# lisanhu/LongReadMapper

Measured on AMD Instinct MI355X. Metric: aligned Gbp/sec, higher is better.
Workload: dtype u8/u64 integer; 1 GPU; E. coli K-12 sized synthetic reference (4641652 bp, 5% planted repeats), 100000 x 10000 bp ont-profile reads per GPU; seed_len=20, thres=300, gact_T=320, gact_O=120, gact_W=128, reads_per_gpu=100000, read_len=10000, streams=3, sa_sampled=1, parallelism=reads sharded, index replicated (1 RCCL bcast)

## Files before the change

longreadmapper_amd/csrc/index_image.hip:

```cpp
#include <hip/hip_runtime.h>
#include <cstdio>
#include <cstdlib>
#include <cstring>
#include <new>
#include <vector>
#include <algorithm>
#include <omp.h>
#include "lrm_hip_util.h"
#include "extend_stage.h"

static inline uint64_t align256(uint64_t x) { return (x + 255ull) & ~255ull; }
#define LRM_LCX_MAX 4096

enum { S_OCC, S_LC, S_LCX, S_SA, S_CONTENT, S_MTA, N_SECTIONS };
struct Section { uint64_t LrmBlobHeader::*off; uint64_t elem; uint64_t (*count)(const LrmBlobHeader &); };
static const Section k_sections[N_SECTIONS] = {
    {&LrmBlobHeader::off_occ, sizeof(LrmOccBlock), [](const LrmBlobHeader &h) { return h.n_blocks; }},
    {&LrmBlobHeader::off_lc, 8, [](const LrmBlobHeader &h) { return h.lc_entries; }},
    {&LrmBlobHeader::off_lcx, 24, [](const LrmBlobHeader &) { return (uint64_t) LRM_LCX_MAX; }},
    {&LrmBlobHeader::off_sa, 8, [](const LrmBlobHeader &h) { return h.sa_len; }},
    {&LrmBlobHeader::off_content, 1, [](const LrmBlobHeader &h) { return h.con_len + 1; }},
    {&LrmBlobHeader::off_mta, sizeof(LrmMtaDev), [](const LrmBlobHeader &h) { return (uint64_t) (h.mta_len > 0 ? h.mta_len : 1); }},
};
static inline uint64_t section_bytes(const LrmBlobHeader &h, int s) { return k_sections[s].elem * k_sections[s].count(h); }
// ... 357 lines not shown
                                const char *content, uint64_t con_len, const lrm_mta_entry *mta, int mta_len, int device) {
    return lrm_index_upload_one(out, fmi, lch, sa, content, con_len, mta, mta_len, device, nullptr);
}

extern "C" int lrm_index_pack_device(const lrm_dna_fmi *fmi, const lrm_lc_hash *lch, const lrm_sa_mem *sa,
                                     const char *content, uint64_t con_len, const lrm_mta_entry *mta, int mta_len,
                                     void *d_blob, uint64_t blob_bytes, int device) {
    return lrm_index_pack_device_opt(fmi, lch, sa, content, con_len, mta, mta_len, d_blob, blob_bytes, device, nullptr);
}
extern "C" int lrm_index_pack_device_opt(const lrm_dna_fmi *fmi, const lrm_lc_hash *lch, const lrm_sa_mem *sa,
                                         const char *content, uint64_t con_len, const lrm_mta_entry *mta, int mta_len,
                                         void *d_blob, uint64_t blob_bytes, int device, const lrm_index_options *opt) {
    if (!fmi || !lch || !d_blob) { lrm_set_error("null argument"); return -1; }
    if (lrm_require_device(device)) return -1;
    BlobPacker pk;
    if (pk.init(fmi, lch, sa, content, con_len, mta, mta_len, opt)) return -1;
    if (blob_bytes < pk.h.total_bytes) { lrm_set_error("device buffer too small for the image"); return -1; }
    return stream_image(pk, d_blob);
}

extern "C" int lrm_index_get_tables(const lrm_index *idx, lrm_index_tables *out) {
    if (!idx || !out) { lrm_set_error("lrm_index_get_tables: null argument"); return -1; }
    memset(out, 0, sizeof(*out));
    const LrmIndexView &v = idx->view;
    uint64_t bytes = 0;
    if (v.lcl) {
        out->lc_long = v.hl; out->lc_pair = v.lcl_pair; out->lc_entry_bytes = v.lcl_kbits ? 5 : 8;
        bytes += ((v.lcl_pair ? 2ull : 1ull) << (2 * v.hl)) * (uint64_t) out->lc_entry_bytes;
        if (v.lclx) bytes += (v.lclx_mask + 1) * 16;
    }
    if (v.core) { out->lc_core = 1; bytes += 64ull << 26; }
    if (v.sd) {
        out->seed_table_len = v.sd_len; out->seed_table_share = v.sd_f; out->seed_table_bits = v.sd_bits;
        out->seed_table_slot_bytes = v.sd_slot; out->seed_table_count_bits = v.sd_cbits;
        out->seed_table_side_entries = idx->sd_side_entries;
        bytes += (64ull << v.sd_bits) + (v.sdx_mask + 1) * 16;
    }
    out->derived_bytes = bytes;
    return 0;
}

extern "C" void lrm_index_free(lrm_index *idx) {
    if (!idx) return;
    for (int r = 1; r < idx->n_peers && idx->peers; ++r) lrm_index_free(idx->peers[r]);
    delete[] idx->peers;
    (void) hipSetDevice(idx->device);
    lrm_host_ctx_free(idx);
    lrm_bs_free_index(idx);
    if (idx->d_lcl) (void) hipFree(idx->d_lcl);
    if (idx->d_lclx) (void) hipFree(idx->d_lclx);
    if (idx->d_core) (void) hipFree(idx->d_core);
    if (idx->d_sd) (void) hipFree(idx->d_sd);
    if (idx->d_sdx) (void) hipFree(idx->d_sdx);
    if (idx->owns_blob && idx->d_blob) (void) hipFree(idx->d_blob);
    delete idx;
}
```

longreadmapper_amd/csrc/index_tables.hip:

```cpp
#include <hip/hip_runtime.h>
#include <cstdio>
#include "seed_index_dev.h"

__device__ __forceinline__ uint64_t lcl_entry(const LrmIndexView &ix, int hl, uint64_t code) {
    const int ext = hl - ix.hlen;
    uint64_t k, l;
    lc_lookup(ix, code >> (2 * ext), k, l);
    if (k == 0 && l == 0) return 0;
    for (int i = ext - 1; i >= 0 && k <= l; --i) {
        const uint32_t c = (uint32_t) (code >> (2 * i)) & 3u;
        uint64_t ra, rb;
        occ_lf2(ix, c, k - 1, l, ra, rb);
        k = ra + 1;
        l = rb;
    }
    if (k > l) return 0;
    const uint64_t cnt = l - k + 1;
    return cnt >= 0xFFFFFFull ? (0xFFFFFFull << 40) : (k | (cnt << 40));
}

__global__ __launch_bounds__(256) void lcl_build_kernel(LrmIndexView ix, int hl, int pair, int kbits, uint64_t *__restrict__ out,
                                                        uint64_t slot0, uint64_t *__restrict__ ovf, uint64_t ovf_cap,
                                                        unsigned long long *__restrict__ n_ovf) {
    const uint64_t slot = slot0 + (uint64_t) blockIdx.x * 256 + threadIdx.x;
// ... 105 lines not shown
            const uint32_t at = atomicAdd(reinterpret_cast<uint32_t *>(line) + 15, 1u) & 0xFFu;
            if (at >= 250u) atomicAdd(n_ovf, 1ull << 40);
            if (at >= 10u) atomicOr(reinterpret_cast<uint32_t *>(line) + 15, 1u << (8u + sd_filter_bit((uint32_t) key.tag)));
            if (at < 10u) {
                uint16_t *h = reinterpret_cast<uint16_t *>(line) + 3 * at;
                h[0] = (uint16_t) v; h[1] = (uint16_t) (v >> 16); h[2] = (uint16_t) (v >> 32);
                placed = true;
            }
        }
        if (!placed) to_side = true;
    }
    if (to_side) {
        const unsigned long long at = atomicAdd(n_ovf, 1ull);
        if (at < ovf_cap) { ovf[2 * at] = code; ovf[2 * at + 1] = side; }
    }
}

__global__ __launch_bounds__(256) void sd_clear_kernel(ulonglong2 *__restrict__ p, uint64_t n16) {
    for (uint64_t i = (uint64_t) blockIdx.x * 256 + threadIdx.x; i < n16; i += (uint64_t) gridDim.x * 256) p[i] = make_ulonglong2(0, 0);
}

struct SdPlan { int f, bits, slot, kbits, cbits; uint64_t bytes; };
static bool sd_plan(const lrm_index *idx, uint64_t free_b, SdPlan *pl) {
    const LrmIndexTune &tu = idx->itune;
    const uint64_t L = idx->view.length;
    const int S = tu.sd_len;
    if (tu.sd == 0 || !idx->cpl_ok || L < 64 || idx->view.con_len != L) return false;
    int kbits = 1;
    while ((1ull << kbits) < L) ++kbits;
    for (int f = 4; f >= 2; f -= 2) {
        if (tu.sd_f && tu.sd_f != f) continue;
        const int slot = f == 4 ? 8 : 6, lf = f == 4 ? 2 : 1;
        const double target = f == 4 ? 2.2 : 6.0;
        int bits = 10;
        while ((double) f * (double) L / (double) (1ull << bits) > target && bits < 34) ++bits;
        if (tu.sd_bits) bits = tu.sd_bits;
        const int CL2 = 2 * (S - f + 1);
        if (bits > CL2) bits = CL2;
        if (bits < 11) bits = 11;
        if (bits < CL2 - 31) bits = CL2 - 31;
        const int tb = lf + 2 * (f - 1) + (CL2 - bits);
        int cbits = (slot == 8 ? 63 : 48) - tb - kbits;
        if (cbits < (tu.sd_bits ? 2 : 4) || tb > 40) continue;
        if (cbits > 24) cbits = 24;
        if (tu.sd_cbits && tu.sd_cbits < cbits) cbits = tu.sd_cbits;
        const uint64_t bytes = 64ull << bits;
        const uint64_t spare = bytes >= (32ull << 30) ? (40ull << 30) : (8ull << 30);
        if (tu.sd < 0 && ((uint64_t) free_b < bytes + bytes / 8 + spare || (tu.lc_long_max >= 13 && bytes > (16ull << 30)))) continue;
        pl->f = f; pl->bits = bits; pl->slot = slot; pl->kbits = kbits; pl->cbits = cbits; pl->bytes = bytes;
        return true;
    }
    return false;
}
static int sd_build(lrm_index *idx, const SdPlan &pl) {
    uint64_t *d = nullptr, *ovf = nullptr, *tab = nullptr;
    uint32_t *claimed = nullptr;
    unsigned long long *n_ovf = nullptr;
    const char *why = "";
    unsigned long long n = 0;
    auto give_up = [&]() {
        if (idx->mtune.verbose) fprintf(stderr, "[lrm] seed table (share %d, 2^%d lines, %d-byte slots) not built: %s (side entries %llu)\n", pl.f, pl.bits, pl.slot, why, n);
        if (d) (void) hipFree(d); if (ovf) (void) hipFree(ovf); if (tab) (void) hipFree(tab); if (n_ovf) (void) hipFree(n_ovf);
        if (claimed) (void) hipFree(claimed);
        (void) hipGetLastError(); return 0; };
    const uint64_t L = idx->view.length, lines = 1ull << pl.bits;
    uint64_t ovf_cap = lines / 4 + 4096;
    if (ovf_cap > (1ull << 30)) ovf_cap = 1ull << 30;
    if (idx->itune.sd_bits) ovf_cap = (uint64_t) pl.f * L + 4096;
    why = "no room for the table";
    if (hipMalloc(&d, pl.bytes) != hipSuccess) { d = nullptr; return give_up(); }
    why = "no room for the overflow list";
    if (hipMalloc(&ovf, ovf_cap * 16) != hipSuccess) { ovf = nullptr; return give_up(); }
    if (hipMalloc(&n_ovf, 8) != hipSuccess) { n_ovf = nullptr; return give_up(); }
    const uint64_t cl_bytes = ((L + 31) / 32 + 1) * 4;
    if (hipMalloc(&claimed, cl_bytes) != hipSuccess) { claimed = nullptr; return give_up(); }
    why = "memset failed";
    if (hipMemset(claimed, 0, cl_bytes) != hipSuccess) return give_up();
    hipLaunchKernelGGL(sd_clear_kernel, dim3(256 * 64), dim3(256), 0, 0, reinterpret_cast<ulonglong2 *>(d), pl.bytes / 16);
    if (hipGetLastError() != hipSuccess || hipMemset(n_ovf, 0, 8) != hipSuccess) return give_up();
    LrmIndexView sdv = idx->view;
    sdv.sd_len = idx->itune.sd_len; sdv.sd_f = pl.f; sdv.sd_bits = pl.bits; sdv.sd_kbits = pl.kbits; sdv.sd_slot = pl.slot; sdv.sd_cbits = pl.cbits;
    const uint64_t chunk = 1ull << 22;
    for (uint64_t b0 = 0, blocks = (L + 255) / 256; b0 < blocks; b0 += chunk) {
        const uint64_t nb = blocks - b0 < chunk ? blocks - b0 : chunk;
        hipLaunchKernelGGL(sd_build_kernel, dim3((uint32_t) nb), dim3(256), 0, 0, idx->view, sdv, d, b0 * 256, claimed, ovf, ovf_cap, n_ovf);
    }
    why = "build kernel failed";
    if (hipDeviceSynchronize() != hipSuccess) { give_up(); lrm_set_error("seed table build failed"); return -1; }
    why = "too many entries beside their lines";
    if (hipMemcpy(&n, n_ovf, 8, hipMemcpyDeviceToHost) != hipSuccess || n > ovf_cap) return give_up();
    uint64_t tslots = 1024;
    while (tslots < 2 * n) tslots <<= 1;
    why = "no room for the side table";
    if (hipMalloc(&tab, tslots * 16) != hipSuccess) { tab = nullptr; return give_up(); }
    if (hipMemset(tab, 0, tslots * 16) != hipSuccess) return give_up();
    if (n) hipLaunchKernelGGL(lclx_build_kernel, dim3((uint32_t) ((n + 255) / 256)), dim3(256), 0, 0, ovf, (uint64_t) n, tab, tslots - 1);
    if (hipDeviceSynchronize() != hipSuccess) { give_up(); lrm_set_error("seed table side build failed"); return -1; }
    (void) hipFree(ovf); (void) hipFree(n_ovf); (void) hipFree(claimed);
    idx->d_sd = d; idx->d_sdx = tab;
    idx->view.sd = d; idx->view.sdx = tab; idx->view.sdx_mask = tslots - 1;
    idx->view.sd_len = sdv.sd_len; idx->view.sd_f = pl.f; idx->view.sd_bits = pl.bits; idx->view.sd_kbits = pl.kbits; idx->view.sd_slot = pl.slot;
    idx->view.sd_cbits = pl.cbits;
    idx->sd_side_entries = n;
    if (idx->mtune.verbose) fprintf(stderr, "[lrm] seed table: %d positions per line, 2^%d lines, %d-byte slots, %d count bits, %llu side entries\n", pl.f, pl.bits, pl.slot, pl.cbits, n);
    return 0;
}

static int lcl_prepare_tables(lrm_index *idx, size_t free_b, bool have_sd);
int lrm_lcl_prepare_index(lrm_index *idx) {
    size_t free_b = 0, total_b = 0;
    if (hipMemGetInfo(&free_b, &total_b) != hipSuccess) { (void) hipGetLastError(); free_b = 0; }
    SdPlan sdp;
    const bool want_sd = sd_plan(idx, free_b, &sdp);
    if (want_sd) { const uint64_t need = sdp.bytes + sdp.bytes / 8; free_b = free_b > need ? free_b - need : 0; }
    const int rc_lcl = lcl_prepare_tables(idx, free_b, want_sd);
    if (rc_lcl) return rc_lcl;
    return want_sd ? sd_build(idx, sdp) : 0;
}

static int lcl_prepare_tables(lrm_index *idx, size_t free_b, bool have_sd) {
    const uint64_t L = idx->view.length;
    int hl = 13, pair = 1, ebytes = 8;
    int kbits = 1;
    while ((1ull << kbits) < L) ++kbits;
    static const struct { int hl, ebytes; uint64_t spare, min_rows; } ladder[] = {
        {17, 5, 40ull << 30, 1ull << 32}, {16, 8, 64ull << 30, 0}, {15, 8, 32ull << 30, 0}, {14, 8, 8ull << 30, 0}};
    for (const auto &c : ladder)
        if (L >= c.min_rows && kbits <= 36 && !(have_sd && c.hl > 16) && (uint64_t) free_b >= (2ull * c.ebytes << (2 * c.hl)) + c.spare) { hl = c.hl; ebytes = c.ebytes; break; }
    const LrmIndexTune &tu = idx->itune;
    if (tu.lc_long_max >= 13 && hl > tu.lc_long_max) { hl = tu.lc_long_max; ebytes = 8; }
    if (tu.lc_long >= 0) { if (tu.lc_long != hl) ebytes = 8; hl = tu.lc_long; }
    if (tu.lc_pair >= 0) pair = tu.lc_pair != 0;
    if (tu.lc_entry_bytes) ebytes = tu.lc_entry_bytes;
    if (!pair || kbits > 36) ebytes = 8;
    if (tu.lc_count_bits && 40 - tu.lc_count_bits >= kbits) kbits = 40 - tu.lc_count_bits;
    if (hl <= idx->view.hlen || hl > 17 || L < 2) return 0;
    uint64_t *d = nullptr, *ovf = nullptr, *tab = nullptr;
    unsigned long long *n_ovf = nullptr;
    const uint64_t slots = (pair ? 2ull : 1ull) << (2 * hl);
    const uint64_t ovf_cap = ebytes == 5 ? (slots / 64 < (64ull << 20) ? slots / 64 + 1024 : (64ull << 20)) : 0;
    auto give_up = [&]() { if (d) (void) hipFree(d); if (ovf) (void) hipFree(ovf); if (tab) (void) hipFree(tab); if (n_ovf) (void) hipFree(n_ovf); (void) hipGetLastError(); };
    if (hipMalloc(&d, slots * (uint64_t) ebytes + 16) != hipSuccess) { d = nullptr; give_up(); return 0; }
    if (ebytes == 5 && (hipMalloc(&ovf, ovf_cap * 16) != hipSuccess || hipMalloc(&n_ovf, 8) != hipSuccess || hipMemset(n_ovf, 0, 8) != hipSuccess)) { give_up(); return 0; }
    const uint64_t chunk = 1ull << 22;
    for (uint64_t b0 = 0, blocks = slots / 256; b0 < blocks; b0 += chunk) {
        const uint64_t nb = blocks - b0 < chunk ? blocks - b0 : chunk;
        hipLaunchKernelGGL(lcl_build_kernel, dim3((uint32_t) nb), dim3(256), 0, 0, idx->view, hl, pair, ebytes == 5 ? kbits : 0, d, b0 * 256,
                           ovf, ovf_cap, n_ovf);
    }
    if (hipDeviceSynchronize() != hipSuccess) { give_up(); lrm_set_error("long lc table build failed"); return -1; }
    uint64_t mask = 0;
    if (ebytes == 5) {
        unsigned long long n = 0;
        if (hipMemcpy(&n, n_ovf, 8, hipMemcpyDeviceToHost) != hipSuccess || n > ovf_cap) { give_up(); return 0; }
        uint64_t tslots = 1024;
        while (tslots < 2 * n) tslots <<= 1;
        mask = tslots - 1;
        if (hipMalloc(&tab, tslots * 16) != hipSuccess || hipMemset(tab, 0, tslots * 16) != hipSuccess) { give_up(); return 0; }
// ... 39 lines not shown
```

longreadmapper_amd/csrc/lrm_api.hip:

```cpp
#include <hip/hip_runtime.h>
#include <cstdarg>
#include <cstdio>
#include <cstdlib>
#include <cstring>
#include <algorithm>
#include <vector>
#include <sched.h>
#include <omp.h>
#include "lrm_hip_util.h"
#include "extend_stage.h"
#include "aln_diff_step.h"
#include "rival_rule.h"

static thread_local char g_err[512] = "";

void lrm_set_error(const char *fmt, ...) {
    va_list ap;
    va_start(ap, fmt);
    vsnprintf(g_err, sizeof(g_err), fmt, ap);
    va_end(ap);
}

extern "C" const char *lrm_last_error(void) { return g_err; }
int lrm_host_threads(void) {
    static const int cap = []() {
        int m = 1 << 20;
        cpu_set_t set;
        if (sched_getaffinity(0, sizeof(set), &set) == 0) { const int c = CPU_COUNT(&set); if (c >= 1 && c < m) m = c; }
        long long quota = -1, period = 0;
        if (FILE *f = fopen("/sys/fs/cgroup/cpu.max", "r")) {
            char q[64];
            if (fscanf(f, "%63s %lld", q, &period) == 2 && strcmp(q, "max") != 0) quota = atoll(q);
            fclose(f);
        } else {
            FILE *fq = fopen("/sys/fs/cgroup/cpu/cpu.cfs_quota_us", "r"), *fp = fopen("/sys/fs/cgroup/cpu/cpu.cfs_period_us", "r");
            if (fq && fp && fscanf(fq, "%lld", &quota) == 1 && fscanf(fp, "%lld", &period) == 1) {} else quota = -1;
            if (fq) fclose(fq);
            if (fp) fclose(fp);
        }
        if (quota > 0 && period > 0) { const int c = (int) (quota / period); if (c >= 1 && c < m) m = c; }
        return m < 1 ? 1 : m;
    }();
    const int m = omp_get_max_threads();
    const int n = m < cap ? m : cap;
    return n < 1 ? 1 : n;
}

extern "C" int lrm_abi_version(void) { return LRM_ABI_VERSION; }

extern "C" int lrm_device_count(void) {
    int n = 0;
    if (hipGetDeviceCount(&n) != hipSuccess) return 0;
    return n;
}

static const char *const k_env_names[] = {
    "LRM_SA_SAMPLED", "LRM_LC_LONG", "LRM_LC_PAIR", "LRM_LC_BYTES", "LRM_LC_CORE", "LRM_LCX_THRESHOLD", "LRM_SD", "LRM_SD_SHARE", "LRM_SD_BITS",
    "LRM_GACT_IMPL", "LRM_SEED_ROUNDS", "LRM_HOST_DENSE", "LRM_HOST_SLICE", "LRM_HOST_SUBS",
    "LRM_HOST_GROUP", "LRM_BS_WAVES", "LRM_SS_ITEMS", "LRM_VOTE_VG", "LRM_VOTE_T1", "LRM_VOTE_U", "LRM_VOTE_LOAD",
    "LRM_HOST_EXT_STREAMS", "LRM_HOST_SEED_STREAMS", "LRM_HOST_VERBOSE", "LRM_VOTE_FAST", "LRM_HOST_SLOTS", "LRM_SS_PAD"};
static_assert(sizeof(k_env_names) / sizeof(k_env_names[0]) <= LrmEnv::MAXV, "LrmEnv too small");

void lrm_env_snapshot(LrmEnv *e) {
    e->n = 0;
    for (const char *name : k_env_names)
        if (const char *v = getenv(name)) {
            e->name[e->n] = name;
            e->val[e->n] = *v ? strtoll(v, nullptr, 0) : 1;
            e->n++;
        }
}
bool LrmEnv::get(const char *key, long long *out) const {
    for (int i = 0; i < n; ++i) if (strcmp(name[i], key) == 0) { *out = val[i]; return true; }
    return false;
}

extern "C" void lrm_index_options_init(lrm_index_options *o) {
    if (!o) return;
    memset(o, 0, sizeof(*o));
    o->struct_size = (uint32_t) sizeof(*o);
    o->lc_long = -1;
    o->lc_pair = -1;
    o->lc_core = -1;
    o->seed_table = -1;
}
extern "C" void lrm_map_options_init(lrm_map_options *o) {
    if (!o) return;
    memset(o, 0, sizeof(*o));
    o->struct_size = (uint32_t) sizeof(*o);
}

static inline bool valid_sa_ratio(long long r) { return r >= 2 && r <= 64 && (r & (r - 1)) == 0; }

void lrm_resolve_index_tune(const lrm_index_options *opt, const LrmEnv &env, LrmIndexTune *t) {
    lrm_index_options o;
    lrm_index_options_init(&o);
    lrm_options_over_defaults(&o, opt);
    t->sa_ratio = valid_sa_ratio(o.sa_sampled) ? o.sa_sampled : 1;
    t->lc_long = o.lc_long; t->lc_long_max = o.lc_long_max; t->lc_pair = o.lc_pair;
    t->lc_entry_bytes = o.lc_entry_bytes == 5 || o.lc_entry_bytes == 8 ? (int) o.lc_entry_bytes : 0;
    t->lc_count_bits = o.lc_count_bits >= 2 && o.lc_count_bits <= 24 ? (int) o.lc_count_bits : 0;
    t->lc_core = o.lc_core;
    t->sd = o.seed_table;
    t->sd_len = o.seed_table_len >= 16 && o.seed_table_len <= 24 ? (int) o.seed_table_len : 20;
    t->sd_f = o.seed_table_share == 2 || o.seed_table_share == 4 ? (int) o.seed_table_share : 0;
    t->sd_bits = o.seed_table_bits >= 4 && o.seed_table_bits <= 32 ? (int) o.seed_table_bits : 0;
    t->sd_cbits = o.seed_table_count_bits >= 2 && o.seed_table_count_bits <= 24 ? (int) o.seed_table_count_bits : 0;
    t->lcx_threshold = o.lcx_threshold >= 1 && o.lcx_threshold <= 0xFFFFFFu ? o.lcx_threshold : 0xFFFFFFull;
    long long v;
    if (env.get("LRM_SA_SAMPLED", &v)) t->sa_ratio = valid_sa_ratio(v) ? (int) v : 1;
    if (env.get("LRM_LC_LONG", &v)) t->lc_long = (int) v;
    if (env.get("LRM_LC_PAIR", &v)) t->lc_pair = v != 0;
    if (env.get("LRM_LC_BYTES", &v) && (v == 5 || v == 8)) t->lc_entry_bytes = (int) v;
    if (env.get("LRM_LC_CORE", &v)) t->lc_core = v != 0;
    if (env.get("LRM_SD", &v)) t->sd = v != 0;
    if (env.get("LRM_SD_SHARE", &v) && (v == 2 || v == 4)) t->sd_f = (int) v;
    if (env.get("LRM_SD_BITS", &v) && v >= 4 && v <= 32) t->sd_bits = (int) v;
    if (env.get("LRM_LCX_THRESHOLD", &v) && v >= 1 && v <= 0xFFFFFFll) t->lcx_threshold = (uint64_t) v;
}

void lrm_resolve_map_tune(const lrm_map_options *opt, const LrmEnv &env, LrmMapTune *t) {
    lrm_map_options o;
    lrm_map_options_init(&o);
    lrm_options_over_defaults(&o, opt);
    memset(t, 0, sizeof(*t));
    t->cigar_text = o.cigar_text != 0;
    t->dense = o.dense_results != 0 || t->cigar_text;
    t->gact_impl = o.gact_impl; t->seed_rounds = o.seed_rounds;
    t->slice_reads = o.slice_reads; t->sub_batches = o.sub_batches; t->group_subs = o.group_subs; t->bs_waves = o.bs_waves;
    t->copy_threads = o.copy_threads <= 16 ? o.copy_threads : 16;
    t->keep_reads = o.keep_reads != 0;
    t->anchored = o.anchored != 0;
    t->anchor_min_len = o.anchor_min_len;
    t->clip = o.clip != 0; t->clip_penalty = o.clip_penalty; t->clip_end_bonus = o.clip_end_bonus;
    t->split = o.split != 0; t->split_min_len = o.split_min_len;
    t->ss_items = 2048; t->vote_vg = 16; t->vote_t1 = LRM_VOTE_T1_LIMIT; t->vote_u = 2; t->vote_load = 50; t->vote_fast = o.vote_exact_only ? 0 : 1;
    t->ext_streams = 2; t->seed_streams = 2;
    long long v;
    if (env.get("LRM_GACT_IMPL", &v)) t->gact_impl = (int) v;
    if (env.get("LRM_SEED_ROUNDS", &v)) t->seed_rounds = (int) v;
    if (env.get("LRM_HOST_DENSE", &v)) t->dense = v != 0 || t->cigar_text;
    if (env.get("LRM_HOST_SLICE", &v) && v >= 1) t->slice_reads = (uint32_t) v;
    if (env.get("LRM_HOST_SUBS", &v) && v >= 1) t->sub_batches = (uint32_t) v;
    if (env.get("LRM_HOST_GROUP", &v) && v >= 1) t->group_subs = (uint32_t) v;
    if (env.get("LRM_BS_WAVES", &v) && v >= 1) t->bs_waves = (uint32_t) v;
    if (env.get("LRM_SS_ITEMS", &v) && (v == 1024 || v == 2048 || v == 4096)) t->ss_items = (uint32_t) v;
    if (env.get("LRM_SS_PAD", &v) && v >= 0 && v <= 60000) t->ss_lds_pad = (uint32_t) v;
    if (env.get("LRM_VOTE_VG", &v) && v >= 1 && v <= 64) t->vote_vg = (uint32_t) v;
    if (env.get("LRM_VOTE_T1", &v) && v >= 0 && v <= LRM_VOTE_T1_LIMIT) t->vote_t1 = (uint32_t) v;
    if (env.get("LRM_VOTE_U", &v)) t->vote_u = (uint32_t) v;
    if (env.get("LRM_VOTE_LOAD", &v) && v >= 10 && v <= 95) t->vote_load = (uint32_t) v;
    if (env.get("LRM_VOTE_FAST", &v)) t->vote_fast = v != 0;
    if (env.get("LRM_HOST_EXT_STREAMS", &v) && v >= 1 && v <= 4) t->ext_streams = (int) v;
    if (env.get("LRM_HOST_SEED_STREAMS", &v) && v >= 1 && v <= 3) t->seed_streams = (int) v;
    if (env.get("LRM_HOST_VERBOSE", &v)) t->verbose = v != 0;
}

int lrm_require_device(int device) {
    int n = 0;
    hipError_t e = hipGetDeviceCount(&n);
    if (e != hipSuccess || n <= 0) {
        lrm_set_error("no HIP device available (%s): liblrm_accel has no CPU fallback", e == hipSuccess ? "count 0" : hipGetErrorString(e));
        return -1;
    }
    if (device < 0 || device >= n) { lrm_set_error("device %d out of range (have %d)", device, n); return -1; }
    HIPCHK(hipSetDevice(device));
    return 0;
}

void lrm_call_map_tune(const lrm_index *ix, const lrm_map_options *opt, LrmMapTune *out) {
// ... 395 lines not shown
```

longreadmapper_amd/csrc/lrm_internal.h:

```cpp
#pragma once
#include <stddef.h>
#include <stdint.h>
#include <stdlib.h>
#include <string.h>
#include "../../include/lrm_accel.h"

#define LRM_BLOB_MAGIC 0x4c524d424c4f4232ull
#define LRM_OCC_ROWS 64

struct LrmOccEntry {
    uint64_t cnt;
    uint64_t mask;
};
struct LrmOccBlock { LrmOccEntry sym[4]; };
static_assert(sizeof(LrmOccBlock) == 64, "occ block must be one 64-B line");

struct LrmMtaDev { uint64_t offset, seq_len; };

struct LrmBlobHeader {
    uint64_t magic, version;
    uint64_t length;
    uint64_t c4[4];
    uint64_t dollar_row;
    uint64_t n_blocks;
    uint64_t lc_entries;
    uint64_t sa_len, con_len;
    uint64_t off_occ, off_lc, off_sa, off_content, off_mta;
    uint64_t total_bytes;
    int32_t hlen, mta_len;
    uint64_t off_lcx, n_lcx;
    uint64_t sa_ratio;
    uint64_t reserved[10];
};
static_assert(sizeof(LrmBlobHeader) == 256, "header is 256 B");

struct LrmIndexView {
    const LrmOccBlock *occ;
    const uint64_t *lc;
    const uint64_t *lcx;
    uint64_t n_lcx;
    const uint64_t *sa;
    const char *content;
    const LrmMtaDev *mta;
    uint64_t length, dollar_row, sa_len, con_len;
    uint64_t c4[4];
    int32_t hlen, mta_len;
    const uint64_t *lcl;
    int32_t hl;
    int32_t sa_shift;
    int32_t lcl_pair;
    int32_t lcl_kbits;
    const uint64_t *core;
    const uint64_t *lclx;
    uint64_t lclx_mask;
    const uint64_t *sd;
    const uint64_t *sdx;
    uint64_t sdx_mask;
    int32_t sd_len;
    int32_t sd_f;
    int32_t sd_bits;
    int32_t sd_kbits;
    int32_t sd_slot;
    int32_t sd_cbits;
};

struct LrmEnv {
    static constexpr int MAXV = 32;
    const char *name[MAXV];
    long long val[MAXV];
    int n;
    bool get(const char *key, long long *out) const;
};
void lrm_env_snapshot(LrmEnv *e);
struct LrmIndexTune {
    int sa_ratio;
    int lc_long, lc_long_max, lc_pair, lc_entry_bytes, lc_count_bits, lc_core;
    int sd, sd_len, sd_f, sd_bits, sd_cbits;
    uint64_t lcx_threshold;
};
struct LrmMapTune {
    int dense, gact_impl, seed_rounds, cigar_text, keep_reads, anchored;
    uint32_t anchor_min_len;
    uint32_t clip, clip_penalty, clip_end_bonus;
    uint32_t split, split_min_len;
    uint32_t slice_reads, sub_batches, group_subs, bs_waves, copy_threads;
    uint32_t ss_items, ss_lds_pad, vote_vg, vote_t1, vote_u, vote_load, vote_fast;
    uint32_t t3_limit, t3_slots;
    int ext_streams, seed_streams, verbose;
};
void lrm_resolve_index_tune(const lrm_index_options *opt, const LrmEnv &env, LrmIndexTune *out);
void lrm_resolve_map_tune(const lrm_map_options *opt, const LrmEnv &env, LrmMapTune *out);
template <typename T>
static inline void lrm_options_over_defaults(T *o, const T *opt) {
    if (opt) memcpy(o, opt, opt->struct_size && opt->struct_size < sizeof(T) ? opt->struct_size : sizeof(T));
}
template <typename T>
static inline void lrm_options_take_fields(T *o, const T *opt, size_t from, size_t to) {
    if (opt && opt->struct_size >= to) memcpy((char *) o + from, (const char *) opt + from, to - from);
}

struct LrmHostCtx;
struct lrm_index;
void lrm_call_map_tune(const lrm_index *ix, const lrm_map_options *opt, LrmMapTune *out);
struct lrm_index {
    void *d_blob;
    uint64_t blob_bytes;
    int owns_blob;
    int device;
    LrmBlobHeader hdr;
    LrmIndexView view;
    uint64_t *d_lcl;
    uint64_t *d_lclx;
    uint64_t *d_core;
    uint64_t *d_sd, *d_sdx;
    uint64_t sd_side_entries;
    uint64_t *d_cpl;
    int cpl_ok;
    uint64_t *d_sas;
    LrmHostCtx *host;
    int n_peers;
    lrm_index **peers;
    LrmEnv env;
    LrmIndexTune itune;
    LrmMapTune mtune;
    uint32_t dbg_t3_limit, dbg_t3_slots;
    uint32_t dbg_mapq_slots;
};

struct LrmPhaseRes {
    uint64_t key1, val1, bucket1;
    uint64_t key2, val2, bucket2;
};

struct LrmDevCounters {
    unsigned long long bs_queue;
    unsigned long long vote_ticket[2];
    unsigned long long seed_traffic[3];
    unsigned long long reserved[2];
    unsigned long long decided_phase0;
    unsigned long long gact_tiles;
    unsigned long long pad[2];
    unsigned long long vote_fast_ticket[2];
    unsigned long long vote_redo_n[2];
    unsigned long long vote_big_n[2];
    unsigned long long vote_big_ticket[2];
    unsigned long long bs_count[7];
};
enum { LRM_BSC_WAVE_TILES = 0, LRM_BSC_P1_MASKED, LRM_BSC_P1_PLAIN, LRM_BSC_P2_FULL, LRM_BSC_P2_WINDOWED, LRM_BSC_P2_SKIPPED,
       LRM_BSC_REFILLS, LRM_BSC_N };
static_assert(offsetof(LrmDevCounters, decided_phase0) == 64 && sizeof(LrmDevCounters) == 216, "counters are addressed by the device as laid out here");
#define LRM_ERR_VOTE_OVERFLOW 1u
#define LRM_VOTE_T1_LIMIT 192
#ifndef LRM_VOTE_T3_SLOTS
#define LRM_VOTE_T3_SLOTS 1024
#endif
#define LRM_VOTE_T3_LIMIT (LRM_VOTE_T3_SLOTS * 3 / 4)
#define LRM_VOTE_GRID 1536
#ifndef LRM_VOTE_FAST_GRID
#define LRM_VOTE_FAST_GRID 1792
#endif
#define LRM_VOTE_KC_CAP 16384

enum LrmKernelId { LRM_K_PACK2BIT = 0, LRM_K_SEED_SEARCH, LRM_K_VOTE, LRM_K_DECIDE,
                   LRM_K_LOCUS, LRM_K_REVCOMP, LRM_K_GACT, LRM_K_PACK_PLANAR, LRM_K_GACT_BS,
                   LRM_K_COUNT };
#define LRM_MAX_TIMED 4096

struct LrmBsScratch {
// ... 148 lines not shown
```

longreadmapper_amd/csrc/seed_kernels.hip:

```cpp
#include <hip/hip_runtime.h>
#include "seed_index_dev.h"

__global__ __launch_bounds__(256) void pack2bit_kernel(const char *__restrict__ reads, uint64_t stride,
                                                       const uint32_t *__restrict__ lens,
                                                       uint8_t *__restrict__ out, uint64_t bytes_per_read,
                                                       uint32_t chunks_per_read, uint64_t n) {
    uint64_t read = blockIdx.x / chunks_per_read;
    uint32_t chunk = blockIdx.x % chunks_per_read;
    if (read >= n) return;
    uint64_t ow = (uint64_t) chunk * 256 + threadIdx.x;
    if (ow * 4 >= bytes_per_read) return;
    uint32_t len = lens[read];
    const uint8_t *r = (const uint8_t *) reads + read * stride;
    uint64_t p = ow * 16;
    uint32_t v = 0;
    if (p + 16 <= len) {
        uint32_t w[4];
        __builtin_memcpy(w, r + p, 16);
#pragma unroll
        for (int t = 0; t < 16; ++t) v |= base_code((w[t >> 2] >> (8 * (t & 3))) & 0xffu) << (2 * t);
    } else {
        for (int t = 0; t < 16; ++t) {
            uint32_t code = (p + t < len) ? base_code(r[p + t]) : 0u;
            v |= code << (2 * t);
        }
    }
    *reinterpret_cast<uint32_t *>(out + read * bytes_per_read + ow * 4) = v;
}

template <int CTRL>
__device__ __forceinline__ uint64_t quad_perm64(uint64_t v) {
    const uint32_t lo = (uint32_t) __builtin_amdgcn_update_dpp(0, (int) (uint32_t) v, CTRL, 0xf, 0xf, true);
    const uint32_t hi = (uint32_t) __builtin_amdgcn_update_dpp(0, (int) (uint32_t) (v >> 32), CTRL, 0xf, 0xf, true);
    return (uint64_t) lo | ((uint64_t) hi << 32);
}
__device__ __forceinline__ void sd_issue_shared(const LrmIndexView &ix, const SdKey &key, ulonglong2 &a, ulonglong2 &b) {
    const uint32_t lane = __lane_id();
    if (ix.sd_f == 4) {
        const uint64_t line = quad_perm64<0x00>(key.line);
        a = *reinterpret_cast<const ulonglong2 *>(ix.sd + line * 8 + (lane & 3u) * 2);
        b = a;
    } else {
        const uint64_t line = quad_perm64<0xA0>(key.line);
        const uint64_t *src = ix.sd + line * 8 + (lane & 1u) * 4;
        a = *reinterpret_cast<const ulonglong2 *>(src);
        b = *reinterpret_cast<const ulonglong2 *>(src + 2);
    }
}
__device__ __forceinline__ int sd_finish_shared(const LrmIndexView &ix, const SdKey &key, uint64_t code, const ulonglong2 &a, const ulonglong2 &b,
                                                uint64_t &k, uint64_t &c, uint32_t *cnt) {
    uint64_t W[8];
    if (ix.sd_f == 4) {
        W[0] = quad_perm64<0x00>(a.x); W[1] = quad_perm64<0x00>(a.y);
        W[2] = quad_perm64<0x55>(a.x); W[3] = quad_perm64<0x55>(a.y);
        W[4] = quad_perm64<0xAA>(a.x); W[5] = quad_perm64<0xAA>(a.y);
        W[6] = quad_perm64<0xFF>(a.x); W[7] = quad_perm64<0xFF>(a.y);
    } else {
        const uint64_t pa = quad_perm64<0xB1>(a.x), pb = quad_perm64<0xB1>(a.y);
        const uint64_t pc = quad_perm64<0xB1>(b.x), pd = quad_perm64<0xB1>(b.y);
        const bool odd = __lane_id() & 1u;
        W[0] = odd ? pa : a.x; W[1] = odd ? pb : a.y; W[2] = odd ? pc : b.x; W[3] = odd ? pd : b.y;
        W[4] = odd ? a.x : pa; W[5] = odd ? a.y : pb; W[6] = odd ? b.x : pc; W[7] = odd ? b.y : pd;
    }
    if (cnt) cnt[0] += 1;
    return sd_search(ix, key, code, W, k, c, cnt);
}

struct __attribute__((aligned(8))) WordPair { uint64_t a, b; };

__device__ __forceinline__ uint64_t read_window(const uint64_t *__restrict__ words, uint32_t j) {
    uint32_t wi = j >> 5, sh = (j & 31) * 2;
    WordPair w;
    __builtin_memcpy(&w, words + wi, sizeof(w));
    return (w.a >> sh) | ((w.b << 1) << (63 - sh));
}

__device__ __forceinline__ void ss_append(uint64_t *s_tot, uint64_t *s_rec, uint32_t *s_q, uint32_t cap_pp, uint32_t ph, uint32_t q, uint64_t k,
                                          uint64_t rr) {
    const uint32_t slot = (uint32_t) atomicAdd(reinterpret_cast<unsigned long long *>(&s_tot[ph]), 1ull | (rr << 32));
    s_rec[ph * cap_pp + slot] = k | (rr << 40);
    s_q[ph * cap_pp + slot] = q;
}

template <int SS_ITEMS, bool COUNT, bool SD48>
__global__ __launch_bounds__(256) __attribute__((amdgpu_waves_per_eu(COUNT ? 1 : 6, 8)))
void seed_search_kernel(LrmIndexView ix, const uint64_t *__restrict__ reads2,
                                                          uint64_t words_per_read,
                                                          const uint32_t *__restrict__ lens,
                                                          const uint8_t *__restrict__ decided, uint64_t n,
                                                          int seed_len, uint32_t thres, int phase_lo, int phase_hi,
                                                          uint32_t cap_q, uint32_t blocks_per_read,
                                                          uint64_t *__restrict__ rec, uint32_t *__restrict__ recq,
                                                          uint32_t *__restrict__ gcnt, uint32_t *__restrict__ ghits,
                                                          LrmDevCounters *counters) {
    __shared__ uint64_t s_rec[SS_ITEMS + 64];
    __shared__ uint32_t s_traffic[3];
    uint32_t my_cnt[2] = {0, 0}, my_seeds = 0;
    if (COUNT && threadIdx.x < 3) s_traffic[threadIdx.x] = 0;
    __shared__ uint32_t s_q[SS_ITEMS + 64];
    __shared__ uint64_t s_tot[64];
    __shared__ uint32_t s_base[64];
    const uint64_t read = blockIdx.x / blocks_per_read;
    const uint32_t chunk = blockIdx.x % blocks_per_read;
    if (read >= n) return;
    if (decided && decided[read]) return;
    const int P = seed_len + 1;
    const uint32_t np = (uint32_t) (phase_hi - phase_lo + 1);
    const uint32_t cap_pp = SS_ITEMS / np + 1;
    const uint32_t tid = threadIdx.x;
    if (tid < np) s_tot[tid] = 0;
    __syncthreads();
    const uint32_t len = lens[read];
    const uint32_t jl = len > (uint32_t) seed_len ? len - (uint32_t) seed_len : 0;
    const uint64_t *words = reads2 + read * words_per_read;
    const bool dense_lanes = (uint32_t) P - np <= 1u;
    const bool shared_lines = ix.sd && seed_len == ix.sd_len && np == (uint32_t) P && phase_lo == 0;
    LrmIndexView ix_nosd = ix;
    ix_nosd.sd = nullptr;
    LrmIndexView ixs = ix;
    if (SD48) { ixs.sd_f = 4; ixs.sd_slot = 8; }
    if (shared_lines) {
        const uint32_t lim = jl < cap_q * np ? jl : cap_q * np;
        const uint32_t np_inv = 0xFFFFFFFFu / np;
        const uint64_t smask = (1ull << (2 * seed_len)) - 1ull;
        const uint32_t dq = 256u / np, dph = 256u % np;
        uint32_t q = __umulhi(chunk * SS_ITEMS + tid, np_inv), ph = chunk * SS_ITEMS + tid - q * np;
        if (ph >= np) { ++q; ph -= np; }
        if (ph >= np) { ++q; ph -= np; }
        struct Look { uint64_t code; SdKey key; ulonglong2 a, b; bool have; };
        auto look = [&](bool real, uint32_t j, uint32_t j0) {
            Look f;
            f.have = real && j < lim;
            f.code = 0;
            f.key.line = 0; f.key.tag = 0; f.key.tb = 0;
            if (real) {
                const uint64_t *wp = words + (j0 >> 5);
                const uint64_t W0 = wp[0], W1 = wp[1], W2 = wp[2];
                const uint32_t rel = j - j0, sh = (rel & 31u) * 2u;
                const uint64_t lo = rel < 32u ? W0 : W1, hi = rel < 32u ? W1 : W2;
                f.code = f.have ? ((lo >> sh) | ((hi << 1) << (63 - sh))) & smask : 0ull;
                f.key = sd_key_of(ixs, f.code, j & (uint32_t) (ixs.sd_f - 1));
            }
            if (SD48) __builtin_assume(f.key.tb <= 32u);
            sd_issue_shared(ixs, f.key, f.a, f.b);
            if (SD48) __builtin_amdgcn_sched_barrier(0);
            return f;
        };
        uint32_t j = chunk * SS_ITEMS + tid;
        uint32_t j0 = (uint32_t) __builtin_amdgcn_readfirstlane((int) (j & ~63u));
        auto take = [&](const Look &f) {
            uint64_t k = 0, l = 0, c = 0, rr;
            const int st = sd_finish_shared(ixs, f.key, f.code, f.a, f.b, k, c, COUNT ? my_cnt : nullptr);
            if (f.have) {
                if (st == 1) rr = c;
                else if (st == 0) rr = 0;
                else rr = seed_one(ix_nosd, f.code, seed_len, j, k, l, COUNT ? my_cnt : nullptr);
                if (COUNT) my_seeds++;
                if (rr > 0 && rr < (uint64_t) thres) ss_append(s_tot, s_rec, s_q, cap_pp, ph, q, k, rr);
            }
        };
        auto step = [&]() {
            j += 256u; j0 += 256u;
            q += dq; ph += dph;
            if (ph >= np) { ++q; ph -= np; }
        };
        if (j0 < lim) {
            const uint32_t left = (lim - j0 + 255u) >> 8;
            const uint32_t n_it = left < (uint32_t) (SS_ITEMS / 256) ? left : (uint32_t) (SS_ITEMS / 256);
            if (SD48) {
                Look fa = look(true, j, j0), fb;
                uint32_t it = 0;
#pragma unroll 1
                do {
                    fb = look(it + 1 < n_it, j + 256u, j0 + 256u);
                    take(fa);
                    step();
                    fa = look(it + 2 < n_it, j + 256u, j0 + 256u);
                    if (it + 1 < n_it) take(fb);
                    step();
                    it += 2;
                } while (it < n_it);
            } else {
#pragma unroll 1
                for (uint32_t it = 0; it < n_it; ++it) {
                    const Look f = look(true, j, j0);
                    take(f);
                    step();
                }
            }
        }
    } else {
    const uint32_t np_inv_g = 0xFFFFFFFFu / np;
#pragma unroll 1
    for (uint32_t it = 0; it < SS_ITEMS / 256; ++it) {
        const uint32_t item = chunk * SS_ITEMS + it * 256 + tid;
        uint32_t q = __umulhi(item, np_inv_g), ph = item - q * np;
        if (ph >= np) { ++q; ph -= np; }
        if (ph >= np) { ++q; ph -= np; }
        uint64_t W[6] = {0, 0, 0, 0, 0, 0};
        uint32_t jw = 0;
        if (dense_lanes) {
            const uint32_t item0 = (uint32_t) __builtin_amdgcn_readfirstlane((int) (item & ~63u));
            const uint32_t q0 = item0 / np;
            if (q0 < cap_q) {
                const uint32_t j0 = (uint32_t) phase_lo + item0 % np + q0 * (uint32_t) P;
                const uint64_t *wp = words + (j0 >> 5);
                jw = j0 & ~31u;
#pragma unroll
                for (int e = 0; e < 6; ++e) W[e] = wp[e];
            }
        }
        if (q >= cap_q) break;
        const uint32_t j = (uint32_t) phase_lo + ph + q * (uint32_t) P;
        if (j >= jl) continue;
        uint64_t win, k, l;
        if (dense_lanes) {
            const uint32_t rel = j - jw, wi = rel >> 5, sh = (rel & 31u) * 2u;
            const uint64_t lo = wi == 0 ? W[0] : wi == 1 ? W[1] : wi == 2 ? W[2] : wi == 3 ? W[3] : W[4];
            const uint64_t hi = wi == 0 ? W[1] : wi == 1 ? W[2] : wi == 2 ? W[3] : wi == 3 ? W[4] : W[5];
            win = (lo >> sh) | ((hi << 1) << (63 - sh));
        } else {
            win = read_window(words, j);
// ... 117 lines not shown
}


int lrm_launch_seed(lrm_index *idx, lrm_workspace *ws, const char *d_reads, uint64_t stride,
                    const uint32_t *d_lens, uint64_t n, uint32_t seed_len,
                    uint32_t thres, lrm_entry *d_best, const LrmMapTune &mt, void *stream_, uint8_t *d_phase_out) {
    hipStream_t stream = (hipStream_t) stream_;
    if (n == 0) return 0;
    ws->seeded_best = nullptr; ws->seeded_n = 0; ws->seeded_phase = 0;
    const int P = (int) seed_len + 1;
    const uint32_t cap_q = ws->cap_q;
    const uint64_t wpr = ws->words_per_read;

    HIPCHK(hipMemsetAsync(ws->d_counters, 0, sizeof(LrmDevCounters), stream));
    HIPCHK(hipMemsetAsync(ws->d_hcount, 0, n * (uint64_t) P * 4, stream));
    HIPCHK(hipMemsetAsync(ws->d_cnt, 0, n * (uint64_t) P * 4, stream));
    ws->n_last = n;
    {
        uint64_t bpr = wpr * 8;
        uint32_t cpr = (uint32_t) ((bpr / 4 + 255) / 256);
        uint32_t grid;
        if (lrm_grid_1d(n * cpr, "pack2bit", &grid)) return -1;
        lrm_time_begin(ws, LRM_K_PACK2BIT, stream);
        hipLaunchKernelGGL(pack2bit_kernel, dim3(grid), dim3(256), 0, stream, d_reads, stride,
                           d_lens, (uint8_t *) ws->d_reads2, bpr, cpr, n);
        lrm_time_end(ws, stream);
    }
    uint32_t tbits = 1;
    while ((1u << tbits) < thres && tbits < 31) tbits++;
    if (((uint64_t) cap_q << tbits) > 0xffffffffull) {
        lrm_set_error("read too long for the vote order key: cap_q %u << %u bits exceeds 32 bits", cap_q, tbits);
        return -1;
    }
    bool single = false;
    {
        const volatile uint64_t *hist = reinterpret_cast<const volatile uint64_t *>(ws->h_err + 2);
        const uint64_t d0 = *hist;
        if (ws->hist_n >= 64 && d0 * 50 < ws->hist_n) single = true;
        if (mt.seed_rounds == 1 || mt.seed_rounds == 2) single = mt.seed_rounds == 1;
        if (P == 1) single = true;
    }
    for (int round = single ? 1 : 0; round < 2; ++round) {
        int lo = round == 0 || single ? 0 : 1;
        int hi = round == 0 ? 0 : P - 1;
        if (lo > hi) break;
        int np = hi - lo + 1;
        const uint8_t *dec = round == 0 || single ? nullptr : ws->d_decided;
        const uint32_t ss_items = mt.ss_items;
        uint32_t bpr = (uint32_t) (((uint64_t) np * cap_q + ss_items - 1) / ss_items);
        uint32_t grid;
        if (lrm_grid_1d(n * bpr, "seed_search", &grid)) return -1;
        lrm_time_begin(ws, LRM_K_SEED_SEARCH, stream);
        const LrmIndexView &v = idx->view;
        const bool sd48 = v.sd && v.sd_f == 4 && v.sd_slot == 8 && 8 + 2 * (v.sd_len - 3) - v.sd_bits <= 32;
        auto sk = ws->counting ? seed_search_kernel<2048, true, false>
                  : sd48 ? (ss_items == 1024u ? seed_search_kernel<1024, false, true> : ss_items == 4096u ? seed_search_kernel<4096, false, true> : seed_search_kernel<2048, false, true>)
                         : (ss_items == 1024u ? seed_search_kernel<1024, false, false> : ss_items == 4096u ? seed_search_kernel<4096, false, false> : seed_search_kernel<2048, false, false>);
        if (ws->counting) bpr = (uint32_t) (((uint64_t) np * cap_q + 2047) / 2048);
        if (ws->counting) grid = (uint32_t) (n * bpr);
        hipLaunchKernelGGL(sk, dim3(grid), dim3(256), mt.ss_lds_pad, stream, idx->view,
                           ws->d_reads2, wpr, d_lens, dec, n, (int) seed_len, thres, lo, hi, cap_q, bpr,
                           ws->d_rec, ws->d_recq, ws->d_cnt, ws->d_hcount, ws->d_counters);
        lrm_time_end(ws, stream);
        const LrmVoteLaunch vl = {dec, n, seed_len, lo, hi, tbits, round, &mt};
        if (lrm_launch_vote(idx, ws, vl, stream)) return -1;
        lrm_time_begin(ws, LRM_K_DECIDE, stream);
        hipLaunchKernelGGL(decide_kernel, dim3((uint32_t) ((n + 255) / 256)), dim3(256), 0, stream, ws->d_phase,
                           d_lens, n, (int) seed_len, single ? 2 : round, ws->d_decided, d_best, ws->d_counters, d_phase_out);
        lrm_time_end(ws, stream);
    }
    HIPCHK(hipMemcpyAsync((void *) (ws->h_err + 2), &ws->d_counters->decided_phase0, 8, hipMemcpyDeviceToHost, stream));
    ws->hist_n = n;
    HIPCHK(hipGetLastError());
    ws->seeded_best = d_best; ws->seeded_n = n;
    ws->seeded_phase = d_phase_out != nullptr && d_phase_out == ws->d_mq_phase;
    return 0;
}

int lrm_launch_debug_seed(lrm_index *idx, const char *d_read, uint32_t len, uint32_t seed_len,
                          uint64_t *d_reads2, uint64_t words, int32_t *d_j, uint64_t *d_rr,
                          uint64_t *d_k, uint64_t *d_l, uint64_t cap, void *stream_) {
    hipStream_t stream = (hipStream_t) stream_;
    const uint32_t P = seed_len + 1;
    uint32_t jl = len > seed_len ? len - seed_len : 0;
    uint32_t cap_q = (jl + P - 1) / P;
    if (cap_q == 0) cap_q = 1;
    if ((uint64_t) cap_q * P > cap) { lrm_set_error("debug seed buffer too small"); return -1; }
    uint64_t bpr = words * 8;
    uint32_t cpr = (uint32_t) ((bpr / 4 + 255) / 256);
    uint32_t *d_len1 = (uint32_t *) (d_reads2 + words);
    HIPCHK(hipMemcpyAsync(d_len1, &len, sizeof(uint32_t), hipMemcpyHostToDevice, stream));
    hipLaunchKernelGGL(pack2bit_kernel, dim3(cpr), dim3(256), 0, stream, d_read, (uint64_t) 0, d_len1,
                       (uint8_t *) d_reads2, bpr, cpr, (uint64_t) 1);
    uint32_t items = cap_q * P;
    hipLaunchKernelGGL(seed_search_debug_kernel, dim3((items + 255) / 256), dim3(256), 0, stream, idx->view,
                       d_reads2, len, (int) seed_len, cap_q, d_j, d_rr, d_k, d_l);
    HIPCHK(hipGetLastError());
    return (int) cap_q;
}
```

Baseline: 63.25 Gbp/s.

## Add occupancy bitmap filter in front of seed table lookups

Builds a compact bitmap over seed-table lines marking which groups of lines are non-empty. The seed search kernel checks this bitmap first and, for keys whose bit is clear, reads from a shared zero region instead of the real table line. A deeper two-stage software pipeline (filter probe, then fetch) is added to hide the extra dependent load. The intent is to cut random DRAM traffic for seeds absent from the reference, at the cost of an additional dependent load, more register pressure, and a build step at index time.

```diff
diff --git a/longreadmapper_amd/csrc/index_image.hip b/longreadmapper_amd/csrc/index_image.hip
--- a/longreadmapper_amd/csrc/index_image.hip
+++ b/longreadmapper_amd/csrc/index_image.hip
@@ -433,6 +433,7 @@
     if (idx->d_core) (void) hipFree(idx->d_core);
     if (idx->d_sd) (void) hipFree(idx->d_sd);
     if (idx->d_sdx) (void) hipFree(idx->d_sdx);
+    if (idx->d_sd_filt) (void) hipFree(idx->d_sd_filt);
     if (idx->owns_blob && idx->d_blob) (void) hipFree(idx->d_blob);
     delete idx;
 }
diff --git a/longreadmapper_amd/csrc/index_tables.hip b/longreadmapper_amd/csrc/index_tables.hip
--- a/longreadmapper_amd/csrc/index_tables.hip
+++ b/longreadmapper_amd/csrc/index_tables.hip
@@ -181,6 +181,7 @@
     }
     return false;
 }
+static void sd_filter_build(lrm_index *idx);
 static int sd_build(lrm_index *idx, const SdPlan &pl) {
     uint64_t *d = nullptr, *ovf = nullptr, *tab = nullptr;
     uint32_t *claimed = nullptr;
@@ -232,7 +233,62 @@
     idx->view.sd_cbits = pl.cbits;
     idx->sd_side_entries = n;
     if (idx->mtune.verbose) fprintf(stderr, "[lrm] seed table: %d positions per line, 2^%d lines, %d-byte slots, %d count bits, %llu side entries\n", pl.f, pl.bits, pl.slot, pl.cbits, n);
+    sd_filter_build(idx);
     return 0;
+}
+
+__global__ __launch_bounds__(256) void sd_filter_kernel(const ulonglong2 *__restrict__ sd, uint64_t lines, uint32_t g,
+                                                        uint32_t *__restrict__ filt) {
+    const uint64_t line = (uint64_t) blockIdx.x * 256 + threadIdx.x;
+    if (line >= lines) return;
+    const ulonglong2 x0 = sd[line * 4], x1 = sd[line * 4 + 1], x2 = sd[line * 4 + 2], x3 = sd[line * 4 + 3];
+    if (((x0.x | x0.y) | (x1.x | x1.y) | (x2.x | x2.y) | (x3.x | x3.y)) == 0) return;
+    const uint64_t bit = line >> g;
+    const uint32_t m = 1u << (bit & 31u);
+    if (!(filt[bit >> 5] & m)) atomicOr(&filt[bit >> 5], m);
+}
+__global__ __launch_bounds__(256) void sd_filter_count_kernel(const uint32_t *__restrict__ filt, uint64_t words,
+                                                              unsigned long long *__restrict__ n_set) {
+    uint32_t c = 0;
+    for (uint64_t i = (uint64_t) blockIdx.x * 256 + threadIdx.x; i < words; i += (uint64_t) gridDim.x * 256) c += __popc(filt[i]);
+    for (int o = 32; o > 0; o >>= 1) c += __shfl_down(c, o, 64);
+    if ((threadIdx.x & 63u) == 0 && c) atomicAdd(n_set, (unsigned long long) c);
+}
+static void sd_filter_build(lrm_index *idx) {
+    const LrmIndexView &v = idx->view;
+    const int kb = idx->itune.sd_filter_kb;
+    if (kb <= 0 || !lrm_sd48_form(v)) return;
+    const uint64_t lines = 1ull << v.sd_bits, max_bits = (uint64_t) kb * 8192;
+    uint32_t g = 0;
+    while ((lines >> g) > max_bits) ++g;
+    const uint64_t bits = lines >> g;
+    if (bits < 512) return;
+    if ((double) v.length / (double) bits > 4.0 * 0.6931471805599453) {
+        if (idx->mtune.verbose) fprintf(stderr, "[lrm] seed filter: not built, %.1f rows per bit at %d KiB\n", (double) v.length / (double) bits, kb);
+        return;
+    }
+    uint32_t *filt = nullptr;
+    unsigned long long *d_n = nullptr, n_set = 0;
+    bool ok = hipMalloc(&filt, bits / 8 + 64) == hipSuccess && hipMalloc(&d_n, 8) == hipSuccess
+              && hipMemset(filt, 0, bits / 8 + 64) == hipSuccess && hipMemset(d_n, 0, 8) == hipSuccess;
+    if (ok) {
+        const uint64_t chunk = 1ull << 30;
+        for (uint64_t l0 = 0; l0 < lines; l0 += chunk) {
+            const uint64_t nl = lines - l0 < chunk ? lines - l0 : chunk;
+            hipLaunchKernelGGL(sd_filter_kernel, dim3((uint32_t) ((nl + 255) / 256)), dim3(256), 0, 0,
+                               reinterpret_cast<const ulonglong2 *>(v.sd) + l0 * 4, nl, g, filt + ((l0 >> g) >> 5));
+        }
+        hipLaunchKernelGGL(sd_filter_count_kernel, dim3(256), dim3(256), 0, 0, filt, bits / 32, d_n);
+        ok = hipDeviceSynchronize() == hipSuccess && hipMemcpy(&n_set, d_n, 8, hipMemcpyDeviceToHost) == hipSuccess;
+    }
+    if (d_n) (void) hipFree(d_n);
+    const bool keep = ok && 2 * n_set <= bits;
+    if (idx->mtune.verbose && ok)
+        fprintf(stderr, "[lrm] seed filter: %llu bytes, one bit per %u lines, %.1f %% of the bits set%s\n", (unsigned long long) (bits / 8), 1u << g,
+                100.0 * (double) n_set / (double) bits, keep ? "" : ": more than half, not kept");
+    if (!keep) { if (filt) (void) hipFree(filt); (void) hipGetLastError(); return; }
+    idx->d_sd_filt = filt;
+    idx->view.sd_filt = filt; idx->view.sd_filt_shift = (int32_t) g;
 }
 
 static int lcl_prepare_tables(lrm_index *idx, size_t free_b, bool have_sd);
diff --git a/longreadmapper_amd/csrc/lrm_api.hip b/longreadmapper_amd/csrc/lrm_api.hip
--- a/longreadmapper_amd/csrc/lrm_api.hip
+++ b/longreadmapper_amd/csrc/lrm_api.hip
@@ -55,7 +55,7 @@
 }
 
 static const char *const k_env_names[] = {
-    "LRM_SA_SAMPLED", "LRM_LC_LONG", "LRM_LC_PAIR", "LRM_LC_BYTES", "LRM_LC_CORE", "LRM_LCX_THRESHOLD", "LRM_SD", "LRM_SD_SHARE", "LRM_SD_BITS",
+    "LRM_SA_SAMPLED", "LRM_LC_LONG", "LRM_LC_PAIR", "LRM_LC_BYTES", "LRM_LC_CORE", "LRM_LCX_THRESHOLD", "LRM_SD", "LRM_SD_SHARE", "LRM_SD_BITS", "LRM_SD_FILTER_KB",
     "LRM_GACT_IMPL", "LRM_SEED_ROUNDS", "LRM_HOST_DENSE", "LRM_HOST_SLICE", "LRM_HOST_SUBS",
     "LRM_HOST_GROUP", "LRM_BS_WAVES", "LRM_SS_ITEMS", "LRM_VOTE_VG", "LRM_VOTE_T1", "LRM_VOTE_U", "LRM_VOTE_LOAD",
     "LRM_HOST_EXT_STREAMS", "LRM_HOST_SEED_STREAMS", "LRM_HOST_VERBOSE", "LRM_VOTE_FAST", "LRM_HOST_SLOTS", "LRM_SS_PAD"};
@@ -116,6 +116,8 @@
     if (env.get("LRM_SD", &v)) t->sd = v != 0;
     if (env.get("LRM_SD_SHARE", &v) && (v == 2 || v == 4)) t->sd_f = (int) v;
     if (env.get("LRM_SD_BITS", &v) && v >= 4 && v <= 32) t->sd_bits = (int) v;
+    t->sd_filter_kb = LRM_SD_FILTER_KB_DEFAULT;
+    if (env.get("LRM_SD_FILTER_KB", &v) && v >= 0 && v <= 65536) t->sd_filter_kb = (int) v;
     if (env.get("LRM_LCX_THRESHOLD", &v) && v >= 1 && v <= 0xFFFFFFll) t->lcx_threshold = (uint64_t) v;
 }
 
diff --git a/longreadmapper_amd/csrc/lrm_internal.h b/longreadmapper_amd/csrc/lrm_internal.h
--- a/longreadmapper_amd/csrc/lrm_internal.h
+++ b/longreadmapper_amd/csrc/lrm_internal.h
@@ -62,7 +62,12 @@
     int32_t sd_kbits;
     int32_t sd_slot;
     int32_t sd_cbits;
-};
+    const uint32_t *sd_filt;
+    int32_t sd_filt_shift;
+};
+static inline bool lrm_sd48_form(const LrmIndexView &v) {
+    return v.sd && v.sd_f == 4 && v.sd_slot == 8 && 8 + 2 * (v.sd_len - 3) - v.sd_bits <= 32;
+}
 
 struct LrmEnv {
     static constexpr int MAXV = 32;
@@ -72,10 +77,12 @@
     bool get(const char *key, long long *out) const;
 };
 void lrm_env_snapshot(LrmEnv *e);
+#define LRM_SD_FILTER_KB_DEFAULT 4096
 struct LrmIndexTune {
     int sa_ratio;
     int lc_long, lc_long_max, lc_pair, lc_entry_bytes, lc_count_bits, lc_core;
     int sd, sd_len, sd_f, sd_bits, sd_cbits;
+    int sd_filter_kb;
     uint64_t lcx_threshold;
 };
 struct LrmMapTune {
@@ -114,6 +121,7 @@
     uint64_t *d_core;
     uint64_t *d_sd, *d_sdx;
     uint64_t sd_side_entries;
+    uint32_t *d_sd_filt;
     uint64_t *d_cpl;
     int cpl_ok;
     uint64_t *d_sas;
diff --git a/longreadmapper_amd/csrc/seed_kernels.hip b/longreadmapper_amd/csrc/seed_kernels.hip
--- a/longreadmapper_amd/csrc/seed_kernels.hip
+++ b/longreadmapper_amd/csrc/seed_kernels.hip
@@ -47,6 +47,21 @@
         b = *reinterpret_cast<const ulonglong2 *>(src + 2);
     }
 }
+__device__ __forceinline__ uint32_t sd_filter_issue(const LrmIndexView &ix, const SdKey &key, bool real, uint32_t &bit) {
+    const uint64_t line = quad_perm64<0x00>(key.line);
+    bit = real ? (uint32_t) (line >> (uint32_t) ix.sd_filt_shift) : 0u;
+    return ix.sd_filt[bit >> 5];
+}
+__device__ __forceinline__ void sd_issue_filtered(const LrmIndexView &ix, const SdKey &key, bool real, uint32_t word, uint32_t bit,
+                                                  ulonglong2 &a, ulonglong2 &b) {
+    const uint32_t lane = __lane_id();
+    const uint64_t line = quad_perm64<0x00>(key.line);
+    const uint64_t *zeros = reinterpret_cast<const uint64_t *>(ix.sd_filt + ((1ull << ix.sd_bits) >> (uint32_t) ix.sd_filt_shift >> 5));
+    const bool pass = real && ((word >> (bit & 31u)) & 1u);
+    const uint64_t *src = pass ? ix.sd + line * 8 : zeros;
+    a = *reinterpret_cast<const ulonglong2 *>(src + (lane & 3u) * 2);
+    b = a;
+}
 __device__ __forceinline__ int sd_finish_shared(const LrmIndexView &ix, const SdKey &key, uint64_t code, const ulonglong2 &a, const ulonglong2 &b,
                                                 uint64_t &k, uint64_t &c, uint32_t *cnt) {
     uint64_t W[8];
@@ -82,7 +97,7 @@
     s_q[ph * cap_pp + slot] = q;
 }
 
-template <int SS_ITEMS, bool COUNT, bool SD48>
+template <int SS_ITEMS, bool COUNT, bool SD48, bool FILT = false>
 __global__ __launch_bounds__(256) __attribute__((amdgpu_waves_per_eu(COUNT ? 1 : 6, 8)))
 void seed_search_kernel(LrmIndexView ix, const uint64_t *__restrict__ reads2,
                                                           uint64_t words_per_read,
@@ -127,7 +142,7 @@
         uint32_t q = __umulhi(chunk * SS_ITEMS + tid, np_inv), ph = chunk * SS_ITEMS + tid - q * np;
         if (ph >= np) { ++q; ph -= np; }
         if (ph >= np) { ++q; ph -= np; }
-        struct Look { uint64_t code; SdKey key; ulonglong2 a, b; bool have; };
+        struct Look { uint64_t code; SdKey key; ulonglong2 a, b; bool have, real; uint32_t word, bit; };
         auto look = [&](bool real, uint32_t j, uint32_t j0) {
             Look f;
             f.have = real && j < lim;
@@ -142,7 +157,9 @@
                 f.key = sd_key_of(ixs, f.code, j & (uint32_t) (ixs.sd_f - 1));
             }
             if (SD48) __builtin_assume(f.key.tb <= 32u);
-            sd_issue_shared(ixs, f.key, f.a, f.b);
+            f.real = real;
+            if (FILT) f.word = sd_filter_issue(ixs, f.key, real, f.bit);
+            else sd_issue_shared(ixs, f.key, f.a, f.b);
             if (SD48) __builtin_amdgcn_sched_barrier(0);
             return f;
         };
@@ -167,7 +184,28 @@
         if (j0 < lim) {
             const uint32_t left = (lim - j0 + 255u) >> 8;
             const uint32_t n_it = left < (uint32_t) (SS_ITEMS / 256) ? left : (uint32_t) (SS_ITEMS / 256);
-            if (SD48) {
+            if (FILT) {
+                auto fetch = [&](Look f) {
+                    sd_issue_filtered(ixs, f.key, f.real, f.word, f.bit, f.a, f.b);
+                    __builtin_amdgcn_sched_barrier(0);
+                    return f;
+                };
+                Look pa = look(true, j, j0), pb = look(1 < n_it, j + 256u, j0 + 256u);
+                Look ga = fetch(pa), gb;
+                uint32_t it = 0;
+#pragma unroll 1
+                do {
+                    pa = look(it + 2 < n_it, j + 512u, j0 + 512u);
+                    gb = fetch(pb);
+                    take(ga);
+                    step();
+                    pb = look(it + 3 < n_it, j + 512u, j0 + 512u);
+                    ga = fetch(pa);
+                    if (it + 1 < n_it) take(gb);
+                    step();
+                    it += 2;
+                } while (it < n_it);
+            } else if (SD48) {
                 Look fa = look(true, j, j0), fb;
                 uint32_t it = 0;
 #pragma unroll 1
@@ -391,8 +429,10 @@
         if (lrm_grid_1d(n * bpr, "seed_search", &grid)) return -1;
         lrm_time_begin(ws, LRM_K_SEED_SEARCH, stream);
         const LrmIndexView &v = idx->view;
-        const bool sd48 = v.sd && v.sd_f == 4 && v.sd_slot == 8 && 8 + 2 * (v.sd_len - 3) - v.sd_bits <= 32;
+        const bool sd48 = lrm_sd48_form(v);
+        const bool filt = sd48 && v.sd_filt;
         auto sk = ws->counting ? seed_search_kernel<2048, true, false>
+                  : filt ? (ss_items == 1024u ? seed_search_kernel<1024, false, true, true> : ss_items == 4096u ? seed_search_kernel<4096, false, true, true> : seed_search_kernel<2048, false, true, true>)
                   : sd48 ? (ss_items == 1024u ? seed_search_kernel<1024, false, true> : ss_items == 4096u ? seed_search_kernel<4096, false, true> : seed_search_kernel<2048, false, true>)
                          : (ss_items == 1024u ? seed_search_kernel<1024, false, false> : ss_items == 4096u ? seed_search_kernel<4096, false, false> : seed_search_kernel<2048, false, false>);
         if (ws->counting) bpr = (uint32_t) (((uint64_t) np * cap_q + 2047) / 2048);
```

New measurement: 66.45 Gbp/s, median of 6. +5.1%, better.
